# Tamnemng/TAM-GCN

Measured on AMD Instinct MI355X. Metric: skeleton clips/sec (fwd+CE+bwd+grad all-reduce+SGD step), N-UCLA 20-joint x 64-frame, higher is better.
Workload: dtype f32 (exact fp32-input MFMA v_mfma_f32_16x16x4_f32 in every GEMM, forward and backward: the reference's arithmetic); 1 GPU; N-UCLA joint stream, 256 clips/GPU x (3,64,20,1), models.ctrgcn.Model fwd+CE+bwd+grad-allreduce+SGD step, train-mode BN; global_batch=256, streams=1, parallelism=dp1, launch=hipgraph, model_streams=0, rehearsal=False, allreduce=one flat bucket after backward

## Files before the change

### tam_gcn_amd/csrc/conv.hip

```cpp
#include "common.h"
#include <stdlib.h>

namespace {

constexpr int BM = 64;
constexpr int BK = 16;
constexpr int BKP = BK + 1;
constexpr int MAXCW = 5;
constexpr int MAXCOLS = 320;
constexpr int NTHREADS = 256;

TG_TRACE_DEFINE(tamgcn_trace_read)

struct ConvArgs {
    SrcDev src;
    int N, K, T_in, V;
    const float* w; const float* bias;
    int M, KT, dil, stride, pad;
    long long ws_m, ws_k, ws_t, w_off;
    int up, wmode;
    float* y; int yctot, ycoff, T_out, T_y, ostride;
    const float* add1; const float* add2; const float* bcast; float bcast_scale;
    SrcDev mask; int has_mask;
    const float* aux; const float* aux_center; int auxctot, auxcoff;
// ... 658 lines not shown
    if (nch > 2) issue(2);
    wait_vmcnt(npre * nissue);
#pragma unroll
    for (int i = 0; i < (PRO ? 1024 / G_NT : 0); ++i) {
        const int e = tid + i * G_NT;
        if (e < K) { cf[e] = cfr[i][0]; cf[K + e] = cfr[i][1]; cf[2 * K + e] = cfr[i][2]; }
    }
    asm volatile("s_waitcnt lgkmcnt(0)\n\ts_barrier" ::: "memory");
    TG_T(tt1); TG_ACC(0, tt1 - tt0);
    constexpr int NK = BK / 4;
    constexpr int NRD = G_MT + G_CWT * NSRC + (PRO ? NSRC + 1 : 0);
    float fa[2][G_MT], bvs[2][G_CWT];
    float fb[G_CWT], fb2[NSRC == 2 ? G_CWT : 1], fc[3];
    const int cfo = G_NST * STG;
    auto rd = [&](int set, int stage, int kg, int k4) {
        int sb = stage * STG + k4 * 4 * LB, sa = stage * STG + BK * G_PBMAX * NSRC + k4 * aadd, sc = cfo + kg + k4 * 4, sx = k4 * axor;
        asm volatile("" : "+s"(sb), "+s"(sa), "+s"(sc), "+s"(sx));
#pragma unroll
        for (int mt = 0; mt < G_MT; ++mt) fa[set][mt] = smem[sa + (va[mt] ^ sx)];
        if constexpr (PRO && !(TG_KO & 2)) {
            fc[0] = smem[sc + kq]; fc[2] = smem[sc + 2 * K + kq];
            if constexpr (NSRC == 2) fc[1] = smem[sc + K + kq];
        }
#pragma unroll
        for (int cc = 0; cc < G_CWT; ++cc) {
            fb[cc] = smem[sb + vb[cc]];
            if constexpr (NSRC == 2) fb2[cc] = smem[sb + vb[cc] + BK * G_PBMAX];
        }
    };
    typedef float pf2 __attribute__((ext_vector_type(2)));
    const bool relu = a.src.act == 1;
    auto pro = [&](int set) {
        if constexpr (!PRO) {
#pragma unroll
            for (int cc = 0; cc < G_CWT; ++cc) bvs[set][cc] = fb[cc];
        } else if (TG_KO & 2) {
#pragma unroll
            for (int cc = 0; cc < G_CWT; ++cc) bvs[set][cc] = fb[cc] + (NSRC == 2 ? fb2[cc] : 0.f);
        } else {
            const pf2 C1 = {fc[0], fc[0]}, C2 = {fc[1], fc[1]}, C0 = {fc[2], fc[2]};
#pragma unroll
            for (int cc = 0; cc + 1 < G_CWT; cc += 2) {
                pf2 v = {fb[cc], fb[cc + 1]};
                if constexpr (NSRC == 2) v = __builtin_elementwise_fma(C1, v, __builtin_elementwise_fma(C2, (pf2){fb2[cc], fb2[cc + 1]}, C0));
                else v = __builtin_elementwise_fma(C1, v, C0);
                bvs[set][cc] = v[0]; bvs[set][cc + 1] = v[1];
            }
            if constexpr (G_CWT & 1) {
                constexpr int cc = G_CWT - 1;
                if constexpr (NSRC == 2) bvs[set][cc] = fmaf(fc[0], fb[cc], fmaf(fc[1], fb2[cc], fc[2]));
                else bvs[set][cc] = fmaf(fc[0], fb[cc], fc[2]);
            }
            if (relu) {
#pragma unroll
                for (int cc = 0; cc < G_CWT; ++cc) asm("v_max_f32 %0, 0, %0" : "+v"(bvs[set][cc]));
            }
        }
    };
    static_assert((G_MT == 2 || G_MT == 4) && G_CWT == 5, "operand lists below");
#define TG_ACC5(mt_) "+v"(acc[mt_][0]), "+v"(acc[mt_][1]), "+v"(acc[mt_][2]), "+v"(acc[mt_][3]), "+v"(acc[mt_][4])
#define TG_V5(x_) "+v"(x_[0]), "+v"(x_[1]), "+v"(x_[2]), "+v"(x_[3]), "+v"(x_[4])
    auto mm = [&](int cur) {
        if constexpr (G_MT == 2) asm volatile("" : "+v"(fa[cur][0]), "+v"(fa[cur][1]), TG_V5(bvs[cur]) :: "memory");
        else asm volatile("" : "+v"(fa[cur][0]), "+v"(fa[cur][1]), "+v"(fa[cur][2]), "+v"(fa[cur][3]), TG_V5(bvs[cur]) :: "memory");
#pragma unroll
        for (int cc = 0; cc < G_CWT; ++cc)
#pragma unroll
            for (int mt = 0; mt < G_MT; ++mt) acc[mt][cc] = mfma16(fa[cur][mt], bvs[cur][cc], acc[mt][cc]);
    };
    auto fin = [&](int nxt) {
        if constexpr (G_MT == 4) asm volatile("" : TG_ACC5(2), TG_ACC5(3) :: "memory");
        if constexpr (NSRC == 2) asm volatile("" : TG_ACC5(0), TG_ACC5(1), TG_V5(fb), TG_V5(fb2) :: "memory");
        else asm volatile("" : TG_ACC5(0), TG_ACC5(1), TG_V5(fb) :: "memory");
        pro(nxt);
        asm volatile("" : TG_V5(bvs[nxt]));
    };
#undef TG_ACC5
#undef TG_V5
    wait_vmcnt((npre - 1) * nissue);
    asm volatile("s_waitcnt lgkmcnt(0)\n\ts_barrier" ::: "memory");
    rd(0, 0, 0, 0);
    pro(0);
    int stg = 0;
    for (int c = 0; c + 1 < nch; ++c) {
        const int k0 = c * BK;
#pragma unroll
        for (int s_ = 0; s_ + 1 < NK; ++s_) {
            rd((s_ & 1) ^ 1, stg, k0, s_ + 1);
            mm(s_ & 1);
            fin((s_ & 1) ^ 1);
        }
        wait_vmcnt(c + 2 < nch ? nissue : 0);
        asm volatile("s_waitcnt lgkmcnt(0)\n\ts_barrier" ::: "memory");
        if (c + 3 < nch) issue(c + 3);
        stg = stg == G_NST - 1 ? 0 : stg + 1;
        rd(NK & 1, stg, k0 + BK, 0);
        mm((NK - 1) & 1);
        fin(NK & 1);
    }
    {
        const int k0 = (nch - 1) * BK;
#pragma unroll
        for (int s_ = 0; s_ < NK; ++s_) {
            if (s_ + 1 < NK) rd((s_ & 1) ^ 1, stg, k0, s_ + 1);
            mm(s_ & 1);
            if (s_ + 1 < NK) fin((s_ & 1) ^ 1);
        }
    }
    TG_T(tg0);

#if TG_KO & 1
    {
        float ssum = 0.f;
        for (int mt = 0; mt < G_MT; ++mt)
            for (int c = 0; c < G_CWT; ++c) ssum += acc[mt][c][0] + acc[mt][c][1] + acc[mt][c][2] + acc[mt][c][3];
        if (ssum == 123.456f) a.y[tid] = ssum;
        return;
    }
#endif
    constexpr int PT = G_CWT * 64 + 4, RP = 32;
    float* Tt = smem;
    if (a.stats_part) {
        for (int e = tid; e < 2 * 4 * BM; e += G_NT) Ss[e] = 0.f;
    }
    for (int r0 = 0; r0 < G_BMT; r0 += RP) {
        __syncthreads();
#pragma unroll
        for (int mt = 0; mt < G_MT; ++mt) {
            const int rl = wm * (G_MT * 16) + mt * 16 - r0;
            if (rl >= 0 && rl < RP) {
#pragma unroll
                for (int c = 0; c < G_CWT; ++c) {
                    const int col = (wn * G_CWT + c) * 16 + j;
#pragma unroll
                    for (int r = 0; r < 4; ++r) Tt[(rl + kq * 4 + r) * PT + col] = acc[mt][c][r];
                }
            }
        }
        __syncthreads();
        staged_rows<G_NT>(a, Tt, PT, RP, r0, G_BMT, m0, n, t0, ncols, Ss, V, 0);
    }
    if (a.stats_part) {
        __syncthreads();
        if (tid < 2 * G_BMT) {
            int stt = tid / G_BMT, row = tid - stt * G_BMT;
            int m = m0 + row;
            if (m < a.M) a.stats_part[((long long)stt * a.stats_ctot + a.stats_coff + m) * a.nparts + g] = Ss[stt * 4 * BM + row];
        }
    }
    TG_T(tg1); TG_ACC(7, tg1 - tg0); TG_ACC(8, tg1 - tt0); TG_ACC(9, 1);
}


constexpr int GS_BK = 32, GS_NST = 2;

template <int TERMS, bool WM0, int MT>
__global__ __launch_bounds__(G_NT) void conv1x1_glds_split_kernel(const ConvArgs a, int ntt, int nmt) {
    constexpr int GS_MT = MT, GS_BMT = 32 * MT, WROWS = 16 * MT;
    extern __shared__ __attribute__((aligned(16))) float smem[];
    constexpr int BK = GS_BK;
    constexpr int STG = BK * G_PBMAX + BK * GS_BMT;
    constexpr int MAXB = ((BK / 4) * 5 + 7) / 8;
    constexpr int NAP = BK * GS_BMT / 256 / 8;
    constexpr int QR = GS_BMT / 4, RPP = 64 / QR;
    float* cf = smem + GS_NST * STG;
    float* Ss = cf + 3 * a.K;
    float* Bc = Ss + 2 * 4 * BM;

    TG_T(tt0);
    const int tid = threadIdx.x, lane = tid & 63, wave = tid >> 6;
    const int j = lane & 15, kq = lane >> 4, wm = wave >> 2, wn = wave & 3;
    const int V = a.V, K = a.K, LB = a.LB;
    const int rot = ((LB & 31) + 16) & 31;
    int g, mtile;
    {
        const int L = blockIdx.x, ng = a.N * ntt;
        if ((ng & 7) == 0) { const int xcd = L & 7, i = L >> 3; mtile = i % nmt; g = (i / nmt) * 8 + xcd; }
        else { g = L / nmt; mtile = L - g * nmt; }
    }
    const int n = g / ntt, tt = g - n * ntt;
    const int m0 = mtile * GS_BMT, t0 = tt * a.BT;
    const int bt = min(a.BT, a.T_out - t0);
    const int ncols = bt * V;
    const long long TV = (long long)a.T_in * V;

    for (int e = tid; e < K; e += G_NT) {
        int ch = a.src.coff + e;
        cf[e] = a.src.coef ? a.src.coef[ch] : 1.f;
        cf[K + e] = (a.src.coef && a.src.x2) ? a.src.coef[a.src.ctot + ch] : 0.f;
        cf[2 * K + e] = a.src.coef ? a.src.coef[2 * a.src.ctot + ch] : 0.f;
    }
    const bool plain = !a.src.coef;
    const int nsrc = a.src.x2 ? 2 : 1;

    const int NQ = (LB + 63) >> 6, NI1 = (BK / 4) * NQ;
    int b_rel[MAXB], b_dst[MAXB];
    bool b_ok[MAXB], b_on[MAXB];
    int nissue = 0;
#pragma unroll
    for (int i = 0; i < MAXB; ++i) {
        const int id = wave + i * 8;
        const bool idok = id < NI1;
        const int grp = (idok ? id : 0) / NQ, q = (idok ? id : 0) - grp * NQ;
        const int f = q * 256 + lane * 4;
        const int r = f / LB, off = f - r * LB;
        int col = off + (r & 1) * rot;
        if (col >= LB) col -= LB;
        b_ok[i] = idok && r < 4 && col < ncols;
        b_rel[i] = (int)((grp * 4 + r) * TV) + col;
        b_dst[i] = grp * 4 * LB + q * 256;
        b_on[i] = __ballot(b_ok[i]) != 0ull;
        nissue += b_on[i] ? 1 : 0;
    }
    const long long xoff = ((long long)n * a.src.ctot + a.src.coff) * TV + (long long)t0 * V;
    const float* xb1 = a.src.x1 + xoff;
    const float* xb2 = a.src.x2 ? a.src.x2 + xoff : nullptr;
    const int nchk = K / BK;
    int a_rel[NAP], a_dst[NAP];
    bool a_ok[NAP];
#pragma unroll
    for (int i = 0; i < NAP; ++i) {
        const int piece = wave * NAP + i;
        if constexpr (WM0) {
            const int m = piece * 8 + (lane >> 3), q = lane & 7;
            a_ok[i] = m0 + m < a.M;
            a_rel[i] = (m0 + (a_ok[i] ? m : 0)) * (int)a.ws_m + 4 * (q ^ (m & 7));
        } else {
            const int kr = piece * RPP + lane / QR, q = lane % QR;
            const int qs = q ^ ((kr & 1) << 2);
            a_ok[i] = m0 + qs * 4 < a.M;
            a_rel[i] = kr * (int)a.ws_k + (m0 + qs * 4) * (int)a.ws_m;
        }
        a_dst[i] = BK * G_PBMAX + piece * 256;
    }
    nissue += NAP;
    auto issue = [&](int c) {
        float* st = smem + (c % GS_NST) * STG;
        const int k0 = (c % nchk) * BK;
        const float* xb = c < nchk ? xb1 : xb2;
#pragma unroll
        for (int i = 0; i < NAP; ++i)
            if (a_ok[i]) __builtin_amdgcn_global_load_lds((tg_gptr)(a.w + a.w_off + (long long)k0 * a.ws_k + a_rel[i]), (tg_lptr)(st + a_dst[i]), 16, 0, 0);
#pragma unroll
        for (int i = 0; i < MAXB; ++i) {
            if (b_on[i]) {
                const float* gp = xb + (long long)k0 * TV + b_rel[i];
                if (b_ok[i]) __builtin_amdgcn_global_load_lds((tg_gptr)gp, (tg_lptr)(st + b_dst[i]), 16, 0, 0);
            }
        }
    };

    int bslot[G_CWT];
#pragma unroll
    for (int c = 0; c < G_CWT; ++c) {
        int col = (wn * G_CWT + c) * 16 + j;
        if (col >= ncols) col = 0;
        int sl = col - (kq & 1) * rot;
        bslot[c] = sl < 0 ? sl + LB : sl;
    }
    int aoff[GS_MT];
#pragma unroll
    for (int mt = 0; mt < GS_MT; ++mt) {
        const int m = wm * WROWS + mt * 16 + j;
        aoff[mt] = WM0 ? m : (((m >> 2) ^ ((kq & 1) << 2)) << 2) + (m & 3);
    }
    f32x4 acc[GS_MT][G_CWT];
#pragma unroll
    for (int mt = 0; mt < GS_MT; ++mt)
#pragma unroll
        for (int c = 0; c < G_CWT; ++c) acc[mt][c] = (f32x4){0.f, 0.f, 0.f, 0.f};
    float bsum[GS_MT];
#pragma unroll
    for (int mt = 0; mt < GS_MT; ++mt) bsum[mt] = 0.f;

    __syncthreads();
    const int nch = nsrc * nchk;
    issue(0);
    TG_T(tt1); TG_ACC(0, tt1 - tt0);
    for (int c = 0; c < nch; ++c) {
        TG_T(ta);
        asm volatile("s_waitcnt vmcnt(0)" ::: "memory");
        TG_T(tb); TG_ACC(2, tb - ta);
        asm volatile("s_waitcnt lgkmcnt(0)\n\ts_barrier" ::: "memory");
        TG_T(tc); TG_ACC(4, tc - tb);
        if (c + 1 < nch) issue(c + 1);
        TG_T(td); TG_ACC(5, td - tc);
        const float* st = smem + (c % GS_NST) * STG;
        const float* As = st + BK * G_PBMAX;
        const int k0 = (c % nchk) * BK;
        float cs[8], c0[8];
        if (!plain) {
            const float* cc1 = cf + (c < nchk ? 0 : K) + k0 + kq;
#pragma unroll
            for (int e = 0; e < 8; ++e) { cs[e] = cc1[4 * e]; c0[e] = c < nchk ? cf[2 * K + k0 + 4 * e + kq] : 0.f; }
        }
        bf16x8_t ah[GS_MT], al[GS_MT];
#pragma unroll
        for (int mt = 0; mt < GS_MT; ++mt) {
            f32x4 v0, v1;
            if constexpr (WM0) {
                const int m = aoff[mt];
#pragma unroll
                for (int e = 0; e < 4; ++e) { v0[e] = As[m * BK + 4 * (e ^ (m & 7)) + kq]; v1[e] = As[m * BK + 4 * ((e + 4) ^ (m & 7)) + kq]; }
            } else {
#pragma unroll
                for (int e = 0; e < 4; ++e) { v0[e] = As[(4 * e + kq) * GS_BMT + aoff[mt]]; v1[e] = As[(4 * (e + 4) + kq) * GS_BMT + aoff[mt]]; }
            }
            if (!plain) {
#pragma unroll
                for (int e = 0; e < 4; ++e) {
                    bsum[mt] = fmaf(v0[e], c0[e], fmaf(v1[e], c0[e + 4], bsum[mt]));
                    v0[e] *= cs[e]; v1[e] *= cs[e + 4];
                }
            }
            split_bf16x8(v0, v1, ah[mt], al[mt]);
        }
        TG_T(te); TG_ACC(3, te - td);
#pragma unroll
        for (int cc = 0; cc < G_CWT; ++cc) {
            f32x4 v0, v1;
#pragma unroll
            for (int e = 0; e < 4; ++e) { v0[e] = st[(4 * e + kq) * LB + bslot[cc]]; v1[e] = st[(4 * (e + 4) + kq) * LB + bslot[cc]]; }
            bf16x8_t bh, bl;
            split_bf16x8(v0, v1, bh, bl);
#pragma unroll
            for (int mt = 0; mt < GS_MT; ++mt) acc[mt][cc] = mfma_split(ah[mt], al[mt], bh, bl, acc[mt][cc]);
        }
        TG_T(tf); TG_ACC(6, tf - te);
    }
    TG_T(tg0);

    constexpr int PT = G_CWT * 64 + 4, RP = 32;
    float* Tt = smem;
    if (a.stats_part) {
        for (int e = tid; e < 2 * 4 * BM; e += G_NT) Ss[e] = 0.f;
    }
#pragma unroll
    for (int mt = 0; mt < GS_MT; ++mt) {
        float t = bsum[mt];
        t += __shfl_xor(t, 16); t += __shfl_xor(t, 32);
        if (wn == 0 && kq == 0) Bc[wm * WROWS + mt * 16 + j] = t;
    }
    for (int r0 = 0; r0 < GS_BMT; r0 += RP) {
        __syncthreads();
        if (wm * WROWS <= r0 && r0 < wm * WROWS + WROWS) {
            const int mtb = (r0 - wm * WROWS) / 16;
#pragma unroll
            for (int mt2 = 0; mt2 < 2; ++mt2)
#pragma unroll
                for (int c = 0; c < G_CWT; ++c) {
                    const int col = (wn * G_CWT + c) * 16 + j;
#pragma unroll
                    for (int r = 0; r < 4; ++r) {
                        const f32x4 v = (MT == 2 || mtb == 0) ? acc[mt2][c] : acc[(MT == 2 ? 0 : 2) + mt2][c];
                        Tt[(mt2 * 16 + kq * 4 + r) * PT + col] = v[r] + Bc[r0 + mt2 * 16 + kq * 4 + r];
                    }
                }
        }
        __syncthreads();
        staged_rows<G_NT>(a, Tt, PT, RP, r0, GS_BMT, m0, n, t0, ncols, Ss + 0, V, 0);
    }
    if (a.stats_part) {
        __syncthreads();
        if (tid < 2 * GS_BMT) {
            int stt = tid / GS_BMT, row = tid - stt * GS_BMT;
            int m = m0 + row;
            if (m < a.M) a.stats_part[((long long)stt * a.stats_ctot + a.stats_coff + m) * a.nparts + g] = Ss[stt * 4 * BM + row];
        }
    }
    TG_T(tg1); TG_ACC(7, tg1 - tg0); TG_ACC(8, tg1 - tt0); TG_ACC(9, 1);
}

template <int NSRC, int BK>
constexpr size_t glds_lds_bytes(int K, bool pro = true) {
    return sizeof(float) * ((size_t)G_NST * (BK * G_PBMAX * NSRC + BK * G_PA) + (pro ? 3 * (size_t)K : 0) + 2 * 4 * BM);
}

struct ConvPlan { int BT, CW, TIN, lstride, sB, LB, pitchB, ntt, bk, mt, cwt, Vs, Vp, nsl; bool vec, flat; size_t lds; };

static int gcd_i(int a, int b) { while (b) { int t = a % b; a = b; b = t; } return a; }

static int plan_conv(const tamgcn_conv_desc* d, ConvPlan* p) {
    const int V = d->V;
    if (V < 1 || V > MAXCOLS) return -1;
    p->flat = d->KT == 1 && d->stride == 1 && d->up == 1 && d->pad == 0 && d->T_in == d->T_out;
    p->Vs = V; p->nsl = 1;
    if (!p->flat && d->KT > 1 && V > 32 && V % 16 == 0) { p->Vs = 16; p->nsl = V / 16; }
    p->Vp = p->flat ? V : ((p->Vs + 3) & ~3);
    const bool vec_try = d->K <= 1024 && (p->flat || (p->Vp & 3) == 0);
    int BT = MAXCOLS / p->Vs; if (BT < 1) BT = 1;
    if (BT > d->T_out) BT = d->T_out;
    const int q = 4 / gcd_i(V, 4);
    if (p->flat && q > 1 && BT >= q) BT -= BT % q;
    for (;;) {
        p->BT = BT;
        p->lstride = (d->KT == 1) ? d->stride : 1;
        p->sB = (d->KT == 1) ? 1 : d->stride;
        p->TIN = (d->KT == 1) ? BT : (BT - 1) * d->stride + (d->KT - 1) * d->dil + 1;
        p->LB = p->TIN * p->Vp;
        int pitch = p->LB;
        pitch += ((16 - (pitch & 31)) + 32) & 31;
        p->pitchB = pitch;
        p->CW = ceil_div(ceil_div(BT * p->Vs, 16), 4);
        p->vec = false; p->bk = BK;
        bool slots_short = false;
        if (vec_try && (p->LB & 3) == 0) {
            int lb4 = p->LB / 4;
            int bk = (d->KT == 1 && 32 * lb4 <= 10 * NTHREADS) ? 32 : 16;
            if (bk * lb4 <= ((bk == 32) ? 10 : 8) * NTHREADS) { p->vec = true; p->bk = bk; }
            else slots_short = true;
        }
        p->mt = d->M <= 16 ? 1 : d->M <= 32 ? 2 : (d->M % 64 == 0 ? 4 : (d->M % 48 == 0 ? 3 : 4));
        if (d->KT > 1 && p->mt == 4) p->mt = 2;
        p->cwt = p->CW <= 3 ? 3 : 5;
        if (p->vec) {
            size_t avail = (((size_t)d->KT * p->mt * 16 * (p->bk + 2) + 3) & ~(size_t)3) + (size_t)p->bk * pitch;
            if (avail < (size_t)16 * (p->cwt * 64 + 4)) p->vec = false;
        }
        p->lds = p->vec ? sizeof(float) * ((((size_t)d->KT * p->mt * 16 * (p->bk + 2) + 3) & ~(size_t)3) + (size_t)p->bk * pitch +
                                           2 * 4 * BM + 3 * (size_t)d->K)
                        : sizeof(float) * ((size_t)d->KT * BM * (BK + 1) + (size_t)BK * pitch + 2 * 4 * BM);
        if (slots_short && BT > 1) { BT = BT > 4 ? BT - 2 : BT - 1; if (p->flat && q > 1 && BT >= q) BT -= BT % q; continue; }
        if (p->lds <= 64 * 1024 || BT == 1) break;
        BT = (BT + 1) / 2;
        if (p->flat && q > 1 && BT >= q) BT -= BT % q;
    }
    if (!p->vec) { p->Vs = V; p->nsl = 1; if (p->Vp != V) {
        p->Vp = V; p->LB = p->TIN * V; int pitch = p->LB; pitch += ((16 - (pitch & 31)) + 32) & 31; p->pitchB = pitch;
        p->CW = ceil_div(ceil_div(p->BT * V, 16), 4);
        p->lds = sizeof(float) * ((size_t)d->KT * BM * (BK + 1) + (size_t)BK * pitch + 2 * 4 * BM); } }
    if (p->lds > 160 * 1024 || p->CW > MAXCW) return -1;
    p->ntt = ceil_div(d->T_out, p->BT);
    return 0;
}

}


extern "C" int tamgcn_conv_nparts(const tamgcn_conv_desc* d) {
    ConvPlan p;
    if (!d || plan_conv(d, &p)) return -1;
    return d->N * p.ntt * p.nsl;
}

extern "C" int tamgcn_conv(const tamgcn_conv_desc* d, void* stream) {
    TG_CHECK(d && d->src.x1 && d->w && d->y, "tamgcn_conv: null pointer");
    TG_CHECK(d->N > 0 && d->K > 0 && d->M > 0 && d->T_in > 0 && d->T_out > 0 && d->V > 0,
             "tamgcn_conv: bad dims N=%d K=%d M=%d T_in=%d T_out=%d V=%d", d->N, d->K, d->M, d->T_in, d->T_out, d->V);
    TG_CHECK(d->KT >= 1 && d->KT <= 9 && d->dil >= 1 && d->stride >= 1 && d->up >= 1 && d->ostride >= 1,
             "tamgcn_conv: bad taps KT=%d dil=%d stride=%d up=%d", d->KT, d->dil, d->stride, d->up);
    TG_CHECK(d->src.coff + d->K <= d->src.ctot && d->ycoff + d->M <= d->yctot, "tamgcn_conv: channel slice out of range");
    TG_CHECK((d->T_out - 1) * d->ostride < d->T_y, "tamgcn_conv: T_out*ostride exceeds T_y");
    TG_CHECK(!(d->N > 65535), "tamgcn_conv: N too large for grid.z");
    TG_CHECK((long long)d->N * d->yctot * d->T_y * d->V < (1LL << 32), "tamgcn_conv: output tensor exceeds 2^32 elements");
    ConvPlan p;
    TG_CHECK(plan_conv(d, &p) == 0, "tamgcn_conv: no tiling for V=%d KT=%d dil=%d stride=%d", d->V, d->KT, d->dil, d->stride);
    ConvArgs a;
    a.src = make_src(d->src);
    a.N = d->N; a.K = d->K; a.T_in = d->T_in; a.V = d->V;
    a.w = d->w; a.bias = d->bias; a.M = d->M; a.KT = d->KT; a.dil = d->dil; a.stride = d->stride; a.pad = d->pad;
    if (d->wmode == 0) { a.ws_m = (long long)d->K * d->KT; a.ws_k = d->KT; a.ws_t = 1; a.w_off = 0; }
    else { a.ws_m = d->KT; a.ws_k = (long long)d->M * d->KT; a.ws_t = -1; a.w_off = d->KT - 1; }
    a.up = d->up; a.wmode = d->wmode;
    a.y = d->y; a.yctot = d->yctot; a.ycoff = d->ycoff; a.T_out = d->T_out; a.T_y = d->T_y; a.ostride = d->ostride;
    a.add1 = d->add1; a.add2 = d->add2; a.bcast = d->bcast; a.bcast_scale = d->bcast_scale;
    a.has_mask = d->mask != nullptr; a.mask = d->mask ? make_src(*d->mask) : null_src();
    a.aux = d->aux; a.aux_center = d->aux_center; a.auxctot = d->auxctot; a.auxcoff = d->auxcoff;
    TG_CHECK(!d->aux || d->aux_center, "tamgcn_conv: aux needs aux_center");
    a.stats_part = d->stats_part; a.stats_ctot = d->stats_ctot; a.stats_coff = d->stats_coff;
    a.post_coef = d->post_coef; a.post_ctot = d->post_ctot; a.post_act = d->post_act;
    TG_CHECK(!d->post_coef || d->post_ctot >= d->ycoff + d->M, "tamgcn_conv: post_coef has %d channels, need %d", d->post_ctot, d->ycoff + d->M);
    a.nparts = d->N * p.ntt * p.nsl;
    a.BT = p.BT; a.CW = p.CW; a.TIN = p.TIN; a.lstride = p.lstride; a.sB = p.sB; a.LB = p.LB; a.pitchB = p.pitchB;
    a.Vs = p.Vs; a.Vp = p.Vp; a.nsl = p.nsl;
    dim3 grid(p.ntt, ceil_div(d->M, BM), d->N);
    const bool aligned16 = (((uintptr_t)d->src.x1 | (uintptr_t)(d->src.x2 ? d->src.x2 : d->src.x1) | (uintptr_t)d->w) & 15) == 0;
    const bool strided1x1 = d->KT == 1 && d->stride == 2 && d->up == 1 && d->pad == 0 && (d->V & 3) == 0 && d->T_out == (d->T_in - 1) / 2 + 1 &&
                            p.lstride == 2 && p.TIN == p.BT && p.nsl == 1 && p.Vp == d->V && !d->mask && !d->aux;
    const bool glds = p.vec && (p.flat || strided1x1) && d->K % 16 == 0 && p.LB >= 64 && p.LB <= G_PBMAX && (p.LB & 3) == 0 &&
                      aligned16 && (long long)d->K * d->T_in * d->V < (1LL << 30);
    const size_t lds_split = sizeof(float) * ((size_t)GS_NST * (GS_BK * G_PBMAX + GS_BK * 128) + 3 * (size_t)d->K + 2 * 4 * BM + 128);
    const bool big = glds && tamgcn_split_mode() >= 1 && d->src.act == 0 && d->M >= 128 && d->M % 4 == 0 && d->K % GS_BK == 0 &&
                     lds_split <= 160 * 1024 && !d->post_coef && d->wmode == 1 && !d->stats_part;
    if (big) {
        const int nmt = ceil_div(d->M, 128);
        const unsigned nblk = (unsigned)(d->N * p.ntt * nmt);
        static tg_devmask fs = 0;
        tg_allow_lds((const void*)conv1x1_glds_split_kernel<2, false, 4>, 160 * 1024, &fs);
        hipLaunchKernelGGL((conv1x1_glds_split_kernel<2, false, 4>), dim3(nblk), dim3(G_NT), lds_split, (hipStream_t)stream, a, p.ntt, nmt);
        tamgcn_note_kernel("conv1x1_glds_split_kernel<2, false, 4>");
    } else if (glds) {
        const int nmt = ceil_div(d->M, G_BMT);
        const unsigned nblk = (unsigned)(d->N * p.ntt * nmt);
        static int nw_env = -1;
        if (nw_env < 0) { const char* e = getenv("TAMGCN_CONV_WAVES"); nw_env = e ? atoi(e) : 8; }
        const bool pro = d->src.coef || d->src.x2 || d->src.act;
#define TG_GLDS_CASE(NS_, BK_, PRO_, NW_)                                                                                 \
        {                                                                                                                   \
            static tg_devmask fl = 0;                                                                                       \
            const size_t lds = glds_lds_bytes<NS_, BK_>(d->K, PRO_);                                                        \
            tg_allow_lds((const void*)conv1x1_glds_kernel<NS_, BK_, PRO_, NW_>, 160 * 1024, &fl);                           \
            hipLaunchKernelGGL((conv1x1_glds_kernel<NS_, BK_, PRO_, NW_>), dim3(nblk), dim3(NW_ * 64), lds, (hipStream_t)stream, a, p.ntt, nmt); \
            tamgcn_note_kernel("conv1x1_glds_kernel<%d, %d, %s, %d>", NS_, BK_, PRO_ ? "true" : "false", NW_);              \
        }
        if (nw_env != 4) {
            if (d->src.x2) TG_GLDS_CASE(2, 8, true, 8) else if (pro) TG_GLDS_CASE(1, 16, true, 8) else TG_GLDS_CASE(1, 16, false, 8)
        } else {
            if (d->src.x2) TG_GLDS_CASE(2, 8, true, 4) else if (pro) TG_GLDS_CASE(1, 16, true, 4) else TG_GLDS_CASE(1, 16, false, 4)
        }
#undef TG_GLDS_CASE
    } else if (p.vec) {
        dim3 gridv(p.ntt * p.nsl, ceil_div(d->M, 16 * p.mt), d->N);
#define TG_CONV_CASE(BKV_, MT_, CW_)                                                                              \
        if (p.bk == BKV_ && p.mt == MT_ && p.cwt == CW_) {                                                         \
            if (p.lds > 64 * 1024)                                                                                 \
                (void)hipFuncSetAttribute((const void*)conv_kernel_vec<BKV_, MT_, CW_>,                            \
                                          hipFuncAttributeMaxDynamicSharedMemorySize, (int)p.lds);                 \
            hipLaunchKernelGGL((conv_kernel_vec<BKV_, MT_, CW_>), gridv, dim3(NTHREADS), p.lds, (hipStream_t)stream, a); \
            tamgcn_note_kernel("conv_kernel_vec<%d, %d, %d>", BKV_, MT_, CW_);                                      \
        } else
        TG_CONV_CASE(32, 4, 5) TG_CONV_CASE(32, 3, 5) TG_CONV_CASE(32, 2, 5) TG_CONV_CASE(32, 1, 5)
        TG_CONV_CASE(32, 4, 3) TG_CONV_CASE(32, 3, 3) TG_CONV_CASE(32, 2, 3) TG_CONV_CASE(32, 1, 3)
        TG_CONV_CASE(16, 4, 5) TG_CONV_CASE(16, 3, 5) TG_CONV_CASE(16, 2, 5) TG_CONV_CASE(16, 1, 5)
        TG_CONV_CASE(16, 4, 3) TG_CONV_CASE(16, 3, 3) TG_CONV_CASE(16, 2, 3) TG_CONV_CASE(16, 1, 3)
        { tamgcn_set_error("tamgcn_conv: no instantiation bk=%d mt=%d cw=%d", p.bk, p.mt, p.cwt); return -1; }
#undef TG_CONV_CASE
    } else {
        if (p.lds > 64 * 1024) (void)hipFuncSetAttribute((const void*)conv_kernel, hipFuncAttributeMaxDynamicSharedMemorySize, (int)p.lds);
        hipLaunchKernelGGL(conv_kernel, grid, dim3(NTHREADS), p.lds, (hipStream_t)stream, a);
        tamgcn_note_kernel("conv_kernel");
    }
    TG_LAUNCH_CHECK("tamgcn_conv");
    return 0;
}

namespace {

struct WgradArgs {
    SrcDev gy, src;
    int N, M, K, T_in, T_out, V, dil, stride, pad;
    float* part; int nsplit;
    int BT, TIN;
    int PY, PX;
    int n_per;
    int KTG;
};

__device__ __forceinline__ float wg_apply(float x1, float x2, float c1, float c2, float c0, int act) {
    float v = fmaf(c1, x1, fmaf(c2, x2, c0));
    return act == 1 ? fmaxf(v, 0.f) : v;
}

template <bool VEC>
__device__ __forceinline__ void wg_fill(float* tile, int pitch, const float* cf, int rows, int nvalid, int ch0,
                                        const SrcDev& s, long long nbase, long long cs, int T, int V, int f0, int frames) {
    const int tid = threadIdx.x;
    const int len = frames * V;
    if constexpr (VEC) {
        const int l4 = len >> 2;
        for (int e = tid; e < rows * l4; e += NTHREADS) {
            int r = e / l4, c4 = e - r * l4;
            int col = c4 << 2;
            int fr = f0 + col / V;
            float4 o = make_float4(0.f, 0.f, 0.f, 0.f);
            if (r < nvalid && fr >= 0 && fr < T) {
                long long g = nbase + (long long)(ch0 + r) * cs + (long long)f0 * V + col;
                float4 a = *reinterpret_cast<const float4*>(s.x1 + g);
                float4 b = make_float4(0.f, 0.f, 0.f, 0.f);
                if (s.x2) b = *reinterpret_cast<const float4*>(s.x2 + g);
                float c1 = cf[r], c2 = cf[rows + r], c0 = cf[2 * rows + r];
                o.x = wg_apply(a.x, b.x, c1, c2, c0, s.act); o.y = wg_apply(a.y, b.y, c1, c2, c0, s.act);
                o.z = wg_apply(a.z, b.z, c1, c2, c0, s.act); o.w = wg_apply(a.w, b.w, c1, c2, c0, s.act);
            }
            float2* d = reinterpret_cast<float2*>(tile + r * pitch + col);
            d[0] = make_float2(o.x, o.y);
            d[1] = make_float2(o.z, o.w);
        }
    } else {
        const bool rcp_ok = len >= 4 && len <= 1024 && V >= 4 && rows * len < (1 << 20);
        const float rlen = 1.0f / (float)len, rV = 1.0f / (float)V;
        for (int e0 = tid; e0 < rows * len; e0 += 4 * NTHREADS) {
            float v1[4], v2[4]; int rr[4], cc[4]; bool ok[4];
#pragma unroll
            for (int i = 0; i < 4; ++i) {
                const int e = e0 + i * NTHREADS;
                const bool in = e < rows * len;
                const int ee = in ? e : 0;
                const int r = rcp_ok ? tc_like_div(ee, rlen) : ee / len, col = ee - r * len;
                const int fr = f0 + (rcp_ok ? tc_like_div(col, rV) : col / V);
                rr[i] = r; cc[i] = col;
                ok[i] = in && r < nvalid && fr >= 0 && fr < T;
                const long long g = nbase + (long long)(ch0 + (ok[i] ? r : 0)) * cs + (long long)f0 * V + (ok[i] ? col : 0);
                v1[i] = ok[i] ? s.x1[g] : 0.f;
                v2[i] = (ok[i] && s.x2) ? s.x2[g] : 0.f;
            }
#pragma unroll
            for (int i = 0; i < 4; ++i) {
                const int e = e0 + i * NTHREADS;
                if (e < rows * len) tile[rr[i] * pitch + cc[i]] = ok[i] ? wg_apply(v1[i], v2[i], cf[rr[i]], cf[rows + rr[i]], cf[2 * rows + rr[i]], s.act) : 0.f;
            }
        }
    }
}

constexpr int WG_NPF = 6;

template <int KT, int WMT, int WKT, bool VEC, bool PS = false>
__global__ __launch_bounds__(NTHREADS) void wgrad_kernel(const WgradArgs a) {
    extern __shared__ __attribute__((aligned(16))) float smem[];
    constexpr int BMW = PS ? 16 : 2 * WMT * 16, BKW = PS ? 16 : 2 * WKT * 16;
    constexpr bool PF = VEC && (KT == 1 || PS);
    float* Ys = smem;
    float* Xs = Ys + BMW * a.PY;
    float* cfY = Xs + BKW * a.PX;
    float* cfX = cfY + 3 * BMW;
    const int tid = threadIdx.x, lane = tid & 63, wave = tid >> 6;
    const int j = lane & 15, kq = lane >> 4;
    const int wr = PS ? 0 : wave >> 1, wc = PS ? 0 : wave & 1;
    const int k0 = blockIdx.x * BKW, m0 = blockIdx.y * BMW, split = blockIdx.z;
    const int V = a.V, V4 = (V + 3) >> 2;
    const int cpt = (a.T_out + a.BT - 1) / a.BT;
    const int c_begin = split * a.n_per, c_end = min(a.N * cpt, c_begin + a.n_per);
    const int mvalid = min(BMW, a.M - m0), kvalid = min(BKW, a.K - k0);

    for (int e = tid; e < BMW; e += NTHREADS) {
        int ch = a.gy.coff + m0 + e;
        bool ok = e < mvalid && a.gy.coef;
        cfY[e] = ok ? a.gy.coef[ch] : 1.f;
        cfY[BMW + e] = (ok && a.gy.x2) ? a.gy.coef[a.gy.ctot + ch] : 0.f;
        cfY[2 * BMW + e] = ok ? a.gy.coef[2 * a.gy.ctot + ch] : 0.f;
    }
    for (int e = tid; e < BKW; e += NTHREADS) {
        int ch = a.src.coff + k0 + e;
        bool ok = e < kvalid && a.src.coef;
        cfX[e] = ok ? a.src.coef[ch] : 1.f;
        cfX[BKW + e] = (ok && a.src.x2) ? a.src.coef[a.src.ctot + ch] : 0.f;
        cfX[2 * BKW + e] = ok ? a.src.coef[2 * a.src.ctot + ch] : 0.f;
// ... 664 lines not shown
```

Baseline: 9025 clips/s.

## Add persistent 1x1 conv kernel with walkers looping over N×T tiles

Adds a persistent 1x1 conv kernel for the global-load-to-LDS path. When the tile grid exceeds twice the CU count, it launches a capped number of walker blocks, each iterating over several (n, t) tiles. Weight loads and the prologue coefficients are set up once per block, and the LDS staging pipeline keeps running across tile boundaries, with an XCD-aware block-to-tile mapping. BN stats partials are reduced per walker, so nparts changes to the walker count. The trade-off is less parallelism slack and possible load imbalance across walkers.

```diff
diff --git a/tam_gcn_amd/csrc/conv.hip b/tam_gcn_amd/csrc/conv.hip
--- a/tam_gcn_amd/csrc/conv.hip
+++ b/tam_gcn_amd/csrc/conv.hip
@@ -834,6 +834,371 @@
 }
 
 
+constexpr int P_MAXK = 128;
+
+template <int NSRC, int BK, bool PRO>
+__global__ __launch_bounds__(512, 4) void conv1x1_pers_kernel(const ConvArgs a, int ntt, int nmt, int P) {
+    constexpr int NW = 8, G_NT = NW * 64, G_MT = 2;
+    extern __shared__ __attribute__((aligned(16))) float smem[];
+    constexpr int STG = BK * G_PBMAX * NSRC + BK * G_PA;
+    constexpr int NAI = BK / NW;
+    constexpr int MAXB = (NSRC * (BK / 4) * 5 + NW - 1) / NW;
+    float* cf = smem + G_NST * STG;
+    float* Ss = cf + (PRO ? 3 * a.K : 0);
+    float* ec = Ss + 2 * 4 * G_BMT;
+
+    const int tid = threadIdx.x, lane = tid & 63, wave = __builtin_amdgcn_readfirstlane(tid >> 6);
+    const int j = lane & 15, kq = lane >> 4, wm = wave >> 2, wn = wave & 3;
+    const int V = a.V, K = a.K, LB = a.LB;
+    const int rot = ((LB & 31) + 16) & 31;
+    int p, mtile;
+    {
+        const int L = blockIdx.x;
+        if ((P & 7) == 0) { const int xcd = L & 7, i = L >> 3; mtile = i % nmt; p = (i / nmt) * 8 + xcd; }
+        else { p = L / nmt; mtile = L - p * nmt; }
+    }
+    const int NG = a.N * ntt;
+    const int ntile = (NG - p + P - 1) / P;
+    const int m0 = mtile * G_BMT;
+    const int ncols = a.BT * V;
+    const long long TV = (long long)a.T_in * V;
+    const int nch = K / BK, Q = ntile * nch;
+
+    const int NQ = (LB + 63) >> 6;
+    const int ls = a.lstride;
+    const float rV_ = 1.0f / (float)V;
+    const int NI1 = (BK / 4) * NQ;
+    int b_rel[MAXB], b_dst[MAXB];
+    bool b_ok[MAXB], b_on[MAXB];
+    int nissue = 0;
+#pragma unroll
+    for (int i = 0; i < MAXB; ++i) {
+        const int id = wave + i * NW;
+        const bool idok = id < NSRC * NI1;
+        const int src = idok ? id / NI1 : 0;
+        const int rem = id - src * NI1;
+        const int grp = rem / NQ, q = rem - grp * NQ;
+        const int f = q * 256 + lane * 4;
+        const int r = f / LB, off = f - r * LB;
+        int col = off + (r & 1) * rot;
+        if (col >= LB) col -= LB;
+        b_ok[i] = idok && r < 4 && col < ncols;
+        const int scol = ls > 1 ? col + tc_like_div(col, rV_) * (ls - 1) * V : col;
+        b_rel[i] = (int)((grp * 4 + r) * TV) + scol + src * 0x40000000;
+        b_dst[i] = src * (BK * G_PBMAX) + grp * 4 * LB + q * 256;
+        b_on[i] = __ballot(b_ok[i]) != 0ull;
+        nissue += b_on[i] ? 1 : 0;
+    }
+    constexpr int RPP = 256 / BK;
+    constexpr int NAP0 = G_BMT / RPP;
+    const bool wm0 = a.wmode == 0;
+    bool a_ok; const float* wbase; int a_dst0 = 0;
+    if (wm0) {
+        const int ml = lane / (BK / 4), q = lane - ml * (BK / 4);
+        const int m = wave * RPP + ml;
+        const int f = BK == 16 ? (m >> 1) & 3 : (m >> 2) & 1;
+        a_ok = wave < NAP0 && m0 + m < a.M;
+        wbase = a.w + (long long)(m0 + (a_ok ? m : 0)) * a.ws_m + a.w_off + 4 * (q ^ f);
+        a_dst0 = wave * 256;
+    } else {
+        a_ok = m0 + lane < a.M;
+        wbase = a.w + (long long)(m0 + (a_ok ? lane : 0)) * a.ws_m + a.w_off;
+    }
+    const bool a_on = __ballot(a_ok) != 0ull;
+    nissue += wm0 ? (a_on ? 1 : 0) : NAI;
+
+    const long long srcoff = (long long)a.src.coff * TV;
+    auto tile_src = [&](int it, const float* x) {
+        const int g = p + it * P, n = g / ntt, tt = g - n * ntt;
+        return x + (long long)n * a.src.ctot * TV + srcoff + (long long)tt * a.BT * ls * V;
+    };
+    int nx_q = 0, nx_s = 0, nx_c = 0, nx_it = 0;
+    const float* nb1 = tile_src(0, a.src.x1);
+    const float* nb2 = NSRC == 2 ? tile_src(0, a.src.x2) : nullptr;
+    auto issue_next = [&]() {
+        if (nx_q >= Q) return;
+        float* st = smem + nx_s * STG;
+        const int k0 = nx_c * BK;
+        if (wm0) {
+            if (a_on) {
+                if (a_ok) __builtin_amdgcn_global_load_lds((tg_gptr)(wbase + k0), (tg_lptr)(st + BK * G_PBMAX * NSRC + a_dst0), 16, 0, 0);
+            }
+        } else {
+#pragma unroll
+            for (int i = 0; i < NAI; ++i) {
+                const int ka = wave * NAI + i;
+                if (a_ok) __builtin_amdgcn_global_load_lds((tg_gptr)(wbase + (long long)(k0 + ka) * a.ws_k),
+                                                           (tg_lptr)(st + BK * G_PBMAX * NSRC + ka * G_PA), 4, 0, 0);
+            }
+        }
+#pragma unroll
+        for (int i = 0; i < MAXB; ++i) {
+            if (b_on[i]) {
+                const float* base = (NSRC == 2 && (b_rel[i] & 0x40000000)) ? nb2 : nb1;
+                const float* gp = base + (long long)k0 * TV + (b_rel[i] & 0x3fffffff);
+                if (b_ok[i]) __builtin_amdgcn_global_load_lds((tg_gptr)gp, (tg_lptr)(st + b_dst[i]), 16, 0, 0);
+            }
+        }
+        ++nx_q;
+        nx_s = nx_s == G_NST - 1 ? 0 : nx_s + 1;
+        if (++nx_c == nch) {
+            nx_c = 0;
+            if (++nx_it < ntile) { nb1 = tile_src(nx_it, a.src.x1); if (NSRC == 2) nb2 = tile_src(nx_it, a.src.x2); }
+        }
+    };
+
+    int vb[G_CWT], va[G_MT];
+#pragma unroll
+    for (int c = 0; c < G_CWT; ++c) {
+        int col = (wn * G_CWT + c) * 16 + j;
+        if (col >= ncols) col = 0;
+        int sl = col - (kq & 1) * rot;
+        vb[c] = kq * LB + (sl < 0 ? sl + LB : sl);
+    }
+#pragma unroll
+    for (int mt = 0; mt < G_MT; ++mt) {
+        const int m = wm * (G_MT * 16) + mt * 16 + j;
+        const int f = BK == 16 ? (m >> 1) & 3 : (m >> 2) & 1;
+        va[mt] = wm0 ? m * BK + 4 * f + kq : kq * G_PA + m;
+    }
+    const int axor = wm0 ? 4 : 0, aadd = wm0 ? 0 : 4 * G_PA;
+
+    constexpr int NCF = (P_MAXK + G_NT - 1) / G_NT;
+    float cfr[NCF][3];
+#pragma unroll
+    for (int i = 0; i < (PRO ? NCF : 0); ++i) {
+        const int e = tid + i * G_NT, ch = a.src.coff + (e < K ? e : 0);
+        cfr[i][0] = a.src.coef ? a.src.coef[ch] : 1.f;
+        cfr[i][1] = (a.src.coef && a.src.x2) ? a.src.coef[a.src.ctot + ch] : 0.f;
+        cfr[i][2] = a.src.coef ? a.src.coef[2 * a.src.ctot + ch] : 0.f;
+    }
+    float ecr = 0.f;
+    {
+        const int row = tid & 63, kind = tid >> 6, m = m0 + row < a.M ? m0 + row : m0;
+        if (kind == 0) ecr = a.bias ? a.bias[m] : 0.f;
+        else if (kind == 1) ecr = a.post_coef ? a.post_coef[a.ycoff + m] : 1.f;
+        else if (kind == 2) ecr = a.post_coef ? a.post_coef[2 * a.post_ctot + a.ycoff + m] : 0.f;
+    }
+    issue_next(); issue_next(); issue_next();
+    wait_vmcnt(nx_q * nissue);
+#pragma unroll
+    for (int i = 0; i < (PRO ? NCF : 0); ++i) {
+        const int e = tid + i * G_NT;
+        if (e < K) { cf[e] = cfr[i][0]; cf[K + e] = cfr[i][1]; cf[2 * K + e] = cfr[i][2]; }
+    }
+    if (tid < 3 * G_BMT) ec[tid] = ecr;
+    asm volatile("s_waitcnt lgkmcnt(0)\n\ts_barrier" ::: "memory");
+
+    constexpr int NK = BK / 4;
+    f32x4 acc[G_MT][G_CWT];
+    float fa[2][G_MT], bvs[2][G_CWT];
+    float fb[G_CWT], fb2[NSRC == 2 ? G_CWT : 1], fc[3];
+    const int cfo = G_NST * STG;
+    auto rd = [&](int set, int stage, int kg, int k4) {
+        int sb = stage * STG + k4 * 4 * LB, sa = stage * STG + BK * G_PBMAX * NSRC + k4 * aadd, sc = cfo + kg + k4 * 4, sx = k4 * axor;
+        asm volatile("" : "+s"(sb), "+s"(sa), "+s"(sc), "+s"(sx));
+#pragma unroll
+        for (int mt = 0; mt < G_MT; ++mt) fa[set][mt] = smem[sa + (va[mt] ^ sx)];
+        if constexpr (PRO) {
+            fc[0] = smem[sc + kq]; fc[2] = smem[sc + 2 * K + kq];
+            if constexpr (NSRC == 2) fc[1] = smem[sc + K + kq];
+        }
+#pragma unroll
+        for (int cc = 0; cc < G_CWT; ++cc) {
+            fb[cc] = smem[sb + vb[cc]];
+            if constexpr (NSRC == 2) fb2[cc] = smem[sb + vb[cc] + BK * G_PBMAX];
+        }
+    };
+    typedef float pf2 __attribute__((ext_vector_type(2)));
+    const bool relu = a.src.act == 1;
+    auto pro = [&](int set) {
+        if constexpr (!PRO) {
+#pragma unroll
+            for (int cc = 0; cc < G_CWT; ++cc) bvs[set][cc] = fb[cc];
+        } else {
+            const pf2 C1 = {fc[0], fc[0]}, C2 = {fc[1], fc[1]}, C0 = {fc[2], fc[2]};
+#pragma unroll
+            for (int cc = 0; cc + 1 < G_CWT; cc += 2) {
+                pf2 v = {fb[cc], fb[cc + 1]};
+                if constexpr (NSRC == 2) v = __builtin_elementwise_fma(C1, v, __builtin_elementwise_fma(C2, (pf2){fb2[cc], fb2[cc + 1]}, C0));
+                else v = __builtin_elementwise_fma(C1, v, C0);
+                bvs[set][cc] = v[0]; bvs[set][cc + 1] = v[1];
+            }
+            {
+                constexpr int cc = G_CWT - 1;
+                if constexpr (NSRC == 2) bvs[set][cc] = fmaf(fc[0], fb[cc], fmaf(fc[1], fb2[cc], fc[2]));
+                else bvs[set][cc] = fmaf(fc[0], fb[cc], fc[2]);
+            }
+            if (relu) {
+#pragma unroll
+                for (int cc = 0; cc < G_CWT; ++cc) asm("v_max_f32 %0, 0, %0" : "+v"(bvs[set][cc]));
+            }
+        }
+    };
+#define TG_ACC5(mt_) "+v"(acc[mt_][0]), "+v"(acc[mt_][1]), "+v"(acc[mt_][2]), "+v"(acc[mt_][3]), "+v"(acc[mt_][4])
+#define TG_V5(x_) "+v"(x_[0]), "+v"(x_[1]), "+v"(x_[2]), "+v"(x_[3]), "+v"(x_[4])
+    auto mmf = [&](int cur) {
+        asm volatile("" : "+v"(fa[cur][0]), "+v"(fa[cur][1]), TG_V5(bvs[cur]) :: "memory");
+#pragma unroll
+        for (int cc = 0; cc < G_CWT; ++cc)
+#pragma unroll
+            for (int mt = 0; mt < G_MT; ++mt) acc[mt][cc] = mfma16(bvs[cur][cc], fa[cur][mt], acc[mt][cc]);
+    };
+    auto fin = [&](int nxt) {
+        if constexpr (NSRC == 2) asm volatile("" : TG_ACC5(0), TG_ACC5(1), TG_V5(fb), TG_V5(fb2) :: "memory");
+        else asm volatile("" : TG_ACC5(0), TG_ACC5(1), TG_V5(fb) :: "memory");
+        pro(nxt);
+        asm volatile("" : TG_V5(bvs[nxt]));
+    };
+#undef TG_ACC5
+#undef TG_V5
+
+    float s1[G_MT], s2[G_MT];
+#pragma unroll
+    for (int mt = 0; mt < G_MT; ++mt) { s1[mt] = 0.f; s2[mt] = 0.f; }
+    const float plo = a.post_act == 1 ? 0.f : -__builtin_inff();
+    int q = 0, stg = 0;
+    for (int it = 0; it < ntile; ++it) {
+        wait_vmcnt((nx_q - 1 - q) * nissue);
+        asm volatile("s_waitcnt lgkmcnt(0)\n\ts_barrier" ::: "memory");
+        if (it > 0) issue_next();
+#pragma unroll
+        for (int mt = 0; mt < G_MT; ++mt)
+#pragma unroll
+            for (int c = 0; c < G_CWT; ++c) acc[mt][c] = (f32x4){0.f, 0.f, 0.f, 0.f};
+        rd(0, stg, 0, 0);
+        pro(0);
+        for (int c = 0; c + 1 < nch; ++c) {
+            const int k0 = c * BK;
+#pragma unroll
+            for (int s_ = 0; s_ + 1 < NK; ++s_) {
+                rd((s_ & 1) ^ 1, stg, k0, s_ + 1);
+                mmf(s_ & 1);
+                fin((s_ & 1) ^ 1);
+            }
+            wait_vmcnt((nx_q - 2 - q) * nissue);
+            asm volatile("s_waitcnt lgkmcnt(0)\n\ts_barrier" ::: "memory");
+            issue_next();
+            ++q;
+            stg = stg == G_NST - 1 ? 0 : stg + 1;
+            rd(NK & 1, stg, k0 + BK, 0);
+            mmf((NK - 1) & 1);
+            fin(NK & 1);
+        }
+        {
+            const int k0 = (nch - 1) * BK;
+#pragma unroll
+            for (int s_ = 0; s_ < NK; ++s_) {
+                if (s_ + 1 < NK) rd((s_ & 1) ^ 1, stg, k0, s_ + 1);
+                mmf(s_ & 1);
+                if (s_ + 1 < NK) fin((s_ & 1) ^ 1);
+            }
+        }
+        ++q;
+        stg = stg == G_NST - 1 ? 0 : stg + 1;
+
+        const int g = p + it * P, n = g / ntt, t0 = (g - n * ntt) * a.BT;
+        const long long ybo = (long long)n * a.yctot * a.T_y * V + (long long)t0 * a.ostride * V;
+        int ln = lane;
+        asm volatile("" : "+v"(ln));
+        const int ej = ln & 15, ekq = ln >> 4;
+        int yo[G_MT][G_CWT], vo[G_CWT];
+        unsigned okm = 0;
+#pragma unroll
+        for (int cc = 0; cc < G_CWT; ++cc) {
+            const int col = (wn * G_CWT + cc) * 16 + ekq * 4;
+            const bool cok = col < ncols;
+            const int c2 = cok ? col : 0;
+            const int fr = tc_like_div(c2, rV_);
+            vo[cc] = c2 - fr * V;
+#pragma unroll
+            for (int mt = 0; mt < G_MT; ++mt) {
+                const int row = wm * 32 + mt * 16 + ej;
+                const bool ok = cok && m0 + row < a.M;
+                okm |= ok ? 1u << (mt * G_CWT + cc) : 0u;
+                yo[mt][cc] = (a.ycoff + (ok ? m0 + row : m0)) * a.T_y * V + (ok ? fr * a.ostride * V + vo[cc] : 0);
+            }
+        }
+#pragma unroll
+        for (int mt = 0; mt < G_MT; ++mt) {
+            const int row = wm * 32 + mt * 16 + ej;
+            const float bia = ec[row], pc1 = ec[G_BMT + row], pc0 = ec[2 * G_BMT + row];
+#pragma unroll
+            for (int cc = 0; cc < G_CWT; ++cc)
+#pragma unroll
+                for (int r = 0; r < 4; ++r) acc[mt][cc][r] = fmaf(pc1, acc[mt][cc][r] + bia, pc0);
+        }
+        if (a.bcast) {
+            const float* bb = a.bcast + (long long)n * V;
+#pragma unroll
+            for (int mt = 0; mt < G_MT; ++mt) {
+                const int row = wm * 32 + mt * 16 + ej, m = m0 + row < a.M ? m0 + row : m0;
+                f32x4 t[G_CWT];
+#pragma unroll
+                for (int cc = 0; cc < G_CWT; ++cc) t[cc] = *reinterpret_cast<const f32x4*>(bb + m * a.N * V + vo[cc]);
+#pragma unroll
+                for (int cc = 0; cc < G_CWT; ++cc)
+#pragma unroll
+                    for (int r = 0; r < 4; ++r) acc[mt][cc][r] = fmaf(t[cc][r], a.bcast_scale, acc[mt][cc][r]);
+            }
+        }
+#pragma unroll
+        for (int ai = 0; ai < 2; ++ai) {
+            const float* ad = ai == 0 ? a.add1 : a.add2;
+            if (!ad) continue;
+            const float* ab = ad + ybo;
+#pragma unroll
+            for (int mt = 0; mt < G_MT; ++mt) {
+                f32x4 t[G_CWT];
+#pragma unroll
+                for (int cc = 0; cc < G_CWT; ++cc) t[cc] = *reinterpret_cast<const f32x4*>(ab + yo[mt][cc]);
+#pragma unroll
+                for (int cc = 0; cc < G_CWT; ++cc) acc[mt][cc] += t[cc];
+            }
+        }
+#pragma unroll
+        for (int mt = 0; mt < G_MT; ++mt)
+#pragma unroll
+            for (int cc = 0; cc < G_CWT; ++cc) {
+#pragma unroll
+                for (int r = 0; r < 4; ++r) acc[mt][cc][r] = fmaxf(acc[mt][cc][r], plo);
+                if (a.stats_part && (okm >> (mt * G_CWT + cc) & 1u)) {
+                    const f32x4 v = acc[mt][cc];
+                    s1[mt] += (v[0] + v[1]) + (v[2] + v[3]);
+                    s2[mt] = fmaf(v[0], v[0], fmaf(v[1], v[1], fmaf(v[2], v[2], fmaf(v[3], v[3], s2[mt]))));
+                }
+            }
+        float* yb = a.y + ybo;
+#pragma unroll
+        for (int mt = 0; mt < G_MT; ++mt)
+#pragma unroll
+            for (int cc = 0; cc < G_CWT; ++cc)
+                if (okm >> (mt * G_CWT + cc) & 1u) *reinterpret_cast<f32x4*>(yb + yo[mt][cc]) = acc[mt][cc];
+    }
+
+    if (a.stats_part) {
+#pragma unroll
+        for (int mt = 0; mt < G_MT; ++mt) {
+            s1[mt] += __shfl_xor(s1[mt], 16); s1[mt] += __shfl_xor(s1[mt], 32);
+            s2[mt] += __shfl_xor(s2[mt], 16); s2[mt] += __shfl_xor(s2[mt], 32);
+            if (kq == 0) {
+                const int row = wm * 32 + mt * 16 + j;
+                Ss[(0 * 4 + wn) * G_BMT + row] = s1[mt];
+                Ss[(1 * 4 + wn) * G_BMT + row] = s2[mt];
+            }
+        }
+        __syncthreads();
+        if (tid < 2 * G_BMT) {
+            const int st = tid / G_BMT, row = tid - st * G_BMT, m = m0 + row;
+            if (m < a.M) {
+                const float* s = Ss + st * 4 * G_BMT + row;
+                a.stats_part[((long long)st * a.stats_ctot + a.stats_coff + m) * a.nparts + p] = ((s[0] + s[G_BMT]) + s[2 * G_BMT]) + s[3 * G_BMT];
+            }
+        }
+    }
+}
+
+
 constexpr int GS_BK = 32, GS_NST = 2;
 
 template <int TERMS, bool WM0, int MT>
@@ -1116,13 +1481,50 @@
     return 0;
 }
 
+static bool glds_route(const tamgcn_conv_desc* d, const ConvPlan& p) {
+    const bool aligned16 = (((uintptr_t)d->src.x1 | (uintptr_t)(d->src.x2 ? d->src.x2 : d->src.x1) | (uintptr_t)d->w) & 15) == 0;
+    const bool strided1x1 = d->KT == 1 && d->stride == 2 && d->up == 1 && d->pad == 0 && (d->V & 3) == 0 && d->T_out == (d->T_in - 1) / 2 + 1 &&
+                            p.lstride == 2 && p.TIN == p.BT && p.nsl == 1 && p.Vp == d->V && !d->mask && !d->aux;
+    return p.vec && (p.flat || strided1x1) && d->K % 16 == 0 && p.LB >= 64 && p.LB <= G_PBMAX && (p.LB & 3) == 0 &&
+           aligned16 && (long long)d->K * d->T_in * d->V < (1LL << 30);
+}
+
+static int device_cus() {
+    static int cus[64] = {0};
+    int dev = 0;
+    (void)hipGetDevice(&dev);
+    int& c = cus[dev & 63];
+    if (c <= 0) {
+        int v = 0;
+        if (hipDeviceGetAttribute(&v, hipDeviceAttributeMultiprocessorCount, dev) != hipSuccess || v <= 0) v = 256;
+        c = v;
+    }
+    return c;
+}
+
+static int pers_walkers(const tamgcn_conv_desc* d, const ConvPlan& p, bool glds, bool split) {
+#ifdef TG_NO_PERS
+    return 0;
+#endif
+    if (!glds || split || d->src.x2 || d->K > P_MAXK || (d->V & 3) || d->mask || d->aux || d->T_out % p.BT) return 0;
+    if ((long long)d->yctot * d->T_y * d->V >= (1LL << 31) || (long long)d->M * d->N * d->V >= (1LL << 31)) return 0;
+    const int NG = d->N * p.ntt, nmt = ceil_div(d->M, G_BMT);
+    const int cap = 2 * device_cus();
+    if ((long long)NG * nmt <= cap) return 0;
+    const int pmax = cap / nmt;
+    if (pmax < 1) return 0;
+    const int per = ceil_div(NG, pmax);
+    return ceil_div(NG, per);
+}
+
 }
 
 
 extern "C" int tamgcn_conv_nparts(const tamgcn_conv_desc* d) {
     ConvPlan p;
     if (!d || plan_conv(d, &p)) return -1;
-    return d->N * p.ntt * p.nsl;
+    const int pw = pers_walkers(d, p, glds_route(d, p), false);
+    return pw > 0 ? pw : d->N * p.ntt * p.nsl;
 }
 
 extern "C" int tamgcn_conv(const tamgcn_conv_desc* d, void* stream) {
@@ -1156,15 +1558,26 @@
     a.BT = p.BT; a.CW = p.CW; a.TIN = p.TIN; a.lstride = p.lstride; a.sB = p.sB; a.LB = p.LB; a.pitchB = p.pitchB;
     a.Vs = p.Vs; a.Vp = p.Vp; a.nsl = p.nsl;
     dim3 grid(p.ntt, ceil_div(d->M, BM), d->N);
-    const bool aligned16 = (((uintptr_t)d->src.x1 | (uintptr_t)(d->src.x2 ? d->src.x2 : d->src.x1) | (uintptr_t)d->w) & 15) == 0;
-    const bool strided1x1 = d->KT == 1 && d->stride == 2 && d->up == 1 && d->pad == 0 && (d->V & 3) == 0 && d->T_out == (d->T_in - 1) / 2 + 1 &&
-                            p.lstride == 2 && p.TIN == p.BT && p.nsl == 1 && p.Vp == d->V && !d->mask && !d->aux;
-    const bool glds = p.vec && (p.flat || strided1x1) && d->K % 16 == 0 && p.LB >= 64 && p.LB <= G_PBMAX && (p.LB & 3) == 0 &&
-                      aligned16 && (long long)d->K * d->T_in * d->V < (1LL << 30);
+    const bool glds = glds_route(d, p);
     const size_t lds_split = sizeof(float) * ((size_t)GS_NST * (GS_BK * G_PBMAX + GS_BK * 128) + 3 * (size_t)d->K + 2 * 4 * BM + 128);
     const bool big = glds && tamgcn_split_mode() >= 1 && d->src.act == 0 && d->M >= 128 && d->M % 4 == 0 && d->K % GS_BK == 0 &&
                      lds_split <= 160 * 1024 && !d->post_coef && d->wmode == 1 && !d->stats_part;
-    if (big) {
+    const int pw = pers_walkers(d, p, glds, big);
+    if (pw > 0) {
+        const int nmt = ceil_div(d->M, G_BMT);
+        a.nparts = pw;
+        const bool pro = d->src.coef || d->src.x2 || d->src.act;
+#define TG_PERS_CASE(NS_, BK_, PRO_)                                                                                       \
+        {                                                                                                                   \
+            static tg_devmask fl = 0;                                                                                       \
+            const size_t lds = glds_lds_bytes<NS_, BK_>(d->K, PRO_) + 3 * G_BMT * sizeof(float);                            \
+            tg_allow_lds((const void*)conv1x1_pers_kernel<NS_, BK_, PRO_>, 160 * 1024, &fl);                                \
+            hipLaunchKernelGGL((conv1x1_pers_kernel<NS_, BK_, PRO_>), dim3(nmt * pw), dim3(512), lds, (hipStream_t)stream, a, p.ntt, nmt, pw); \
+            tamgcn_note_kernel("conv1x1_pers_kernel<%d, %d, %s>", NS_, BK_, PRO_ ? "true" : "false");                      \
+        }
+        if (pro) TG_PERS_CASE(1, 16, true) else TG_PERS_CASE(1, 16, false)
+#undef TG_PERS_CASE
+    } else if (big) {
         const int nmt = ceil_div(d->M, 128);
         const unsigned nblk = (unsigned)(d->N * p.ntt * nmt);
         static tg_devmask fs = 0;
```

Result: no change. 9039 clips/s, median of 3 (+0.2%).
